# wdc3iii/legged_gym_dev

Hardware: AMD Instinct MI355X
Metric: env-steps/sec (whole node), ANYmal-C flat 4096 envs per GPU (higher is better)
Workload: dtype f32

## Files before the change

legged_gym_dev_amd/csrc/ppo_api.hip:

```cpp
#include <cstdlib>
#include <cstring>
#include <string>
#include <vector>

#include "ppo_device.h"
#include "ppo_mlp_args.h"
#include "ppo_rnn.h"

void lg_set_error(const std::string &s);

extern "C" {
void ppok_gemm_fwd(const GemmArgs *g, int nz, hipStream_t s);
void ppok_gemm_dx(const GemmArgs *g, int nz, hipStream_t s);
void ppok_sync_planes(const PpoDev *P, hipStream_t s);
int ppok_mlp_fwd(const MlpArgs *g, const PpoDev *P, hipStream_t s);
int ppok_mlp_supported(const MlpArgs *g);
int64_t ppok_mlp_frag_elems(int K, int N);
void ppok_mlp_frag_build(const MlpArgs *g, hipStream_t s);
void ppok_gemm_dw(const GemmArgs *g, int nz, hipStream_t s);
void ppok_act_sample(const PpoDev *P, const float *obs, const float *cobs, const float *mu, const float *val, int t,
                     int64_t cnt, int inject, hipStream_t s);
void ppok_process_step(const PpoDev *P, const float *rew, const uint8_t *dones, const uint8_t *tos, int t, hipStream_t s);
void ppok_gae(const PpoDev *P, const float *last_values, hipStream_t s);
void ppok_det_fold(const PpoDev *P, hipStream_t s);
void ppok_adv_normalize(const PpoDev *P, hipStream_t s);
void ppok_gather(const PpoDev *P, int mb, hipStream_t s);
void ppok_randperm(const PpoDev *P, int n, uint64_t update_idx, hipStream_t s);
void ppok_loss(const PpoDev *P, const float *mu, const float *v, float *dmu, float *dval, hipStream_t s);
int ppok_step(const PpoDev *P, int par, const PpoDev *G, int gather_mb, hipStream_t s);
// ... 62 lines not shown
    long long *det_buf;
    int act_code;
    int grads_dirty;
    lg_ctx *env;
    int pp_pending, pp_t, pp_use_tos;
    int params_dirty;
    int fused_act;
    MlpArgs mlp;
    int step, inject;
    int64_t act_count, update_count;
    int Mmax;
    std::vector<void *> allocs;
    int64_t perm_count;
    struct MbSet { float *obs, *critic_obs, *actions, *mu, *scalars; } mbset[2];
    int mb_cur, mb_ready, mb_last;
    lg_ppo_buffers pub;
    Rnn rnn;
};

template <typename T>
static bool palloc(lg_ppo *p, T **out, size_t n) {
    void *q = nullptr;
    size_t bytes = (n ? n : 1) * sizeof(T);
    if (hipMalloc(&q, bytes) != hipSuccess || hipMemset(q, 0, bytes) != hipSuccess) return false;
    p->allocs.push_back(q);
    *out = (T *)q;
    return true;
}
#define PA(ptr, n) do { if (!palloc(p, &(ptr), (n))) { lg_set_error("hipMalloc failed in lg_ppo_create"); lg_ppo_destroy(p); return -100; } } while (0)

// ... 44 lines not shown
        bufs[n] = p->dev.grads + p->dev.num_params; counts[n++] = 2;
    }
    return n;
}
static void reduce_layer_bucket(lg_ppo *p, int l, hipStream_t ready_on) {
    float *bufs[4];
    int64_t counts[4];
    const int n = bucket_extents(p, l, bufs, counts);
    hipStream_t cs = lg_comm_stream_(p->comm);
    (void)hipEventRecord(p->ev_bucket, ready_on);
    (void)hipStreamWaitEvent(cs, p->ev_bucket, 0);
    const int rc = lg_comm_group_allreduce_(p->comm, bufs, counts, n, cs);
    if (rc && !p->comm_rc) p->comm_rc = rc;
}

static void backward(lg_ppo *p, int M, const float *in0, const float *in1, int skip_head = 0) {
    const float *in[2] = {in0, in1};
    auto det_args = [&](GemmArgs &g) {
        g.det_base = p->dev.grads; g.det64 = p->dev.det64; g.det_n = p->dev.num_params + 2;
    };
    const int nl = p->net[0].nl;
    for (int l = nl - 1 - skip_head; l >= 0; --l) {
        GemmArgs g;
        memset(&g, 0, sizeof(g));
        det_args(g);
        for (int z = 0; z < 2; ++z) {
            Net &n = p->net[z];
            g.A[z] = n.dz[l + 1]; g.lda[z] = n.dims[l + 1];
            g.B[z] = l == 0 ? in[z] : n.act[l]; g.ldb[z] = n.dims[l];
            g.C[z] = p->dev.grads + n.w_off[l]; g.ldc[z] = n.dims[l];
            g.M[z] = n.dims[l + 1]; g.N[z] = n.dims[l]; g.K[z] = M;
            if (l == 0 && !p->rnn.H) {
                const int ldp = z == 0 ? p->dev.Op : p->dev.OCp;
                g.ldb[z] = ldp;
                if (ldp != n.dims[0]) { g.N[z] = ldp; g.nstore[z] = n.dims[0]; }
            }
        }
        const bool on_side = p->overlap && l > 0;
        hipStream_t dw_stream = on_side ? p->side : p->stream;
        if (on_side) {
            (void)hipEventRecord(p->ev_dz, p->stream);
            (void)hipStreamWaitEvent(p->side, p->ev_dz, 0);
        }
        ppok_gemm_dw(&g, 2, dw_stream);
        if (p->comm) reduce_layer_bucket(p, l, dw_stream);
        if (l > 0) {
            memset(&g, 0, sizeof(g));
            det_args(g);
            for (int z = 0; z < 2; ++z) {
                Net &n = p->net[z];
                g.A[z] = n.dz[l + 1]; g.lda[z] = n.dims[l + 1];
                g.B[z] = p->dev.params + n.w_off[l]; g.ldb[z] = n.dims[l];
                g.Bpl[z] = p->dev.wpl + n.pl_off[l];
                g.C[z] = n.dz[l]; g.ldc[z] = n.dims[l];
                g.aux[z] = n.act[l]; g.ldaux[z] = n.dims[l];
                g.colsum[z] = p->dev.grads + n.b_off[l - 1];
                g.M[z] = M; g.N[z] = n.dims[l]; g.K[z] = n.dims[l + 1];
// ... 6 lines not shown
    if (p->rnn.H) {
        GemmArgs g;
        memset(&g, 0, sizeof(g));
        for (int z = 0; z < 2; ++z) {
            Net &n = p->net[z];
            g.A[z] = n.dz[1]; g.lda[z] = n.dims[1];
            g.B[z] = p->dev.params + n.w_off[0]; g.ldb[z] = n.dims[0];
            g.Bpl[z] = p->dev.wpl + n.pl_off[0];
            g.C[z] = p->rnn.dh[z]; g.ldc[z] = n.dims[0];
            g.aux[z] = p->rnn.dh[z]; g.ldaux[z] = n.dims[0];
            g.M[z] = M; g.N[z] = n.dims[0]; g.K[z] = n.dims[1];
        }
        g.elu = 0;
        g.pl_stride = p->dev.pl_stride;
        ppok_gemm_dx(&g, 2, p->stream);
    }
    if (p->overlap) {
        (void)hipEventRecord(p->ev_side, p->side);
        (void)hipStreamWaitEvent(p->stream, p->ev_side, 0);
    }
    if (p->comm) {
        const bool rec = p->comm_timing && p->comm_ev_used + 2 <= 2 * 4096;
        if (rec) {
            while (p->comm_ev.size() < p->comm_ev_used + 2) { hipEvent_t e; (void)hipEventCreate(&e); p->comm_ev.push_back(e); }
            (void)hipEventRecord(p->comm_ev[p->comm_ev_used], p->stream);
        }
        (void)hipEventRecord(lg_comm_event_(p->comm), lg_comm_stream_(p->comm));
        (void)hipStreamWaitEvent(p->stream, lg_comm_event_(p->comm), 0);
        if (rec) { (void)hipEventRecord(p->comm_ev[p->comm_ev_used + 1], p->stream); p->comm_ev_used += 2; }
    }
// ... 162 lines not shown
    const int OC = cfg->num_critic_obs > 0 ? cfg->num_critic_obs : O;
    if ((long)N * T % cfg->num_mini_batches != 0 && (long)N * T / cfg->num_mini_batches == 0) { lg_set_error("bad minibatch count"); return -5; }
    const int H = rc ? rc->hidden : 0;
    if (rc) {
        if (rc->type != 0) { lg_set_error("recurrent policy: only rnn_type 'lstm' (0) is implemented"); return -6; }
        if (rc->layers != 1) { lg_set_error("recurrent policy: only rnn_num_layers = 1 is implemented"); return -6; }
        if (H < 32 || H > 512 || H % 32) { lg_set_error("recurrent policy: rnn_hidden_size must be a multiple of 32 in [32, 512]"); return -6; }
    }
    lg_ppo *p = new lg_ppo();
    p->cfg = *cfg;
    memset(&p->rnn, 0, sizeof(p->rnn));
    p->stream = nullptr;
    p->act_code = cfg->activation + 1;
    p->fused_act = getenv("LG_FUSED_ACT") ? atoi(getenv("LG_FUSED_ACT")) : 1;
    p->overlap = getenv("LG_PPO_OVERLAP") ? atoi(getenv("LG_PPO_OVERLAP")) : 1;
    if (hipStreamCreateWithFlags(&p->side, hipStreamNonBlocking) != hipSuccess ||
        hipEventCreateWithFlags(&p->ev_dz, hipEventDisableTiming) != hipSuccess ||
        hipEventCreateWithFlags(&p->ev_side, hipEventDisableTiming) != hipSuccess ||
        hipEventCreateWithFlags(&p->ev_bucket, hipEventDisableTiming) != hipSuccess) {
        lg_set_error("stream/event creation failed"); delete p; return -100;
    }
    p->step = 0; p->inject = 0; p->act_count = 0; p->update_count = 0; p->params_dirty = 1;
    p->comm = nullptr; p->comm_rc = 0; p->comm_timing = 0; p->comm_ev_used = 0;
    p->env = nullptr; p->pp_pending = 0;
    p->perm_count = 0;
    const int R = (int)((long)N * T / cfg->num_mini_batches);
    p->Mmax = R > N ? R : N;

    int64_t off = 0;
    PpoDev &d = p->dev;
    memset(&d, 0, sizeof(d));
    d.off_std = (int)off; off += A;
    for (int z = 0; z < 2; ++z) {
// ... 65 lines not shown
    if (cfg->num_critic_obs > 0) PA(d.st_critic_obs, TN * OC); else d.st_critic_obs = d.st_obs;
    PA(d.st_actions, TN * A); PA(d.st_rewards, TN); PA(d.st_values, TN); PA(d.st_returns, TN); PA(d.st_adv, TN);
    PA(d.st_log_prob, TN); PA(d.st_mu, TN * A); PA(d.st_sigma, A); PA(d.st_dones, TN);
    PA(d.act_actions, (size_t)N * A); PA(d.act_values, N); PA(d.act_log_prob, N); PA(d.act_mu, (size_t)N * A);
    PA(d.stats, 8); PA(d.loss_acc, 4); PA(d.noise, (size_t)N * A); PA(d.perm, TN); PA(d.adv_partial, 4);
    for (int k = 0; k < 2; ++k) {
        lg_ppo::MbSet &m = p->mbset[k];
        PA(m.obs, (size_t)R * d.Op);
        if (cfg->num_critic_obs > 0) PA(m.critic_obs, (size_t)R * d.OCp); else m.critic_obs = m.obs;
        PA(m.actions, (size_t)R * A); PA(m.mu, (size_t)R * A); PA(m.scalars, (size_t)R * 4);
    }
    p->mb_cur = 0; p->mb_ready = -1; p->mb_last = -1;
    d.mb_obs = p->mbset[0].obs; d.mb_critic_obs = p->mbset[0].critic_obs; d.mb_actions = p->mbset[0].actions;
    d.mb_mu = p->mbset[0].mu; d.mb_scalars = p->mbset[0].scalars;
    PA(d.head_part, ppok_head_part_floats());
    PA(d.cur_reward_sum, N); PA(d.cur_episode_len, N); PA(d.ep_stats, 4); PA(d.ep_ring, 200); PA(d.ep_ring_count, 1);
    for (int z = 0; z < 2; ++z) {
        Net &n = p->net[z];
        n.act[0] = nullptr; n.dz[0] = nullptr;
        for (int l = 1; l <= n.nl; ++l) { PA(n.act[l], (size_t)p->Mmax * n.dims[l]); PA(n.dz[l], (size_t)p->Mmax * n.dims[l]); }
    }
    if (H) {
        Rnn &q = p->rnn;
        const size_t NH = (size_t)N * H, Rr = (size_t)R;
        for (int z = 0; z < 2; ++z) {
            PA(q.h[z], NH); PA(q.c[z], NH); PA(q.sv_h[z], TN * H); PA(q.sv_c[z], TN * H); PA(q.tmp_h[z], NH); PA(q.tmp_c[z], NH);
            PA(q.pg[z], Rr * 4 * H); PA(q.gates[z], Rr * 4 * H);
            PA(q.hout[z], Rr * H); PA(q.cout[z], Rr * H); PA(q.hused[z], Rr * H); PA(q.cused[z], Rr * H); PA(q.dh[z], Rr * H);
            PA(q.dc[z], (size_t)q.mbs * H);
        }
// ... 54 lines not shown
    }
    out->hidden = p->rnn.H;
    return 0;
}
int lg_ppo_reset_hidden(lg_ppo *p, const uint8_t *dones) {
    if (!p->rnn.H) { lg_set_error("lg_ppo_reset_hidden: not a recurrent learner"); return -15; }
    flush_rollout_epilogue(p);
    const Rnn &q = p->rnn;
    ppok_lstm_reset(q.h[0], q.c[0], q.h[1], q.c[1], dones, p->cfg.num_envs, q.H, p->stream);
    return launch_ok();
}
int lg_ppo_get_buffers(lg_ppo *p, lg_ppo_buffers *out) { *out = p->pub; return 0; }
int lg_ppo_set_stream(lg_ppo *p, void *s) { p->stream = (hipStream_t)s; return 0; }
int lg_ppo_inject_noise(lg_ppo *p, int enable) { p->inject = enable; return 0; }
int lg_ppo_debug_set_overlap(lg_ppo *p, int v) { p->overlap = v; return 0; }
int lg_ppo_debug_set_fused_act(lg_ppo *p, int v) { p->fused_act = v && p->mlp.wfrag; return 0; }
int lg_ppo_debug_get_fused_act(lg_ppo *p) { return p->fused_act; }
int lg_ppo_debug_set_act_count(lg_ppo *p, long long v) { p->act_count = v; return 0; }

int lg_ppo_param_layout(lg_ppo *p, int64_t *offsets, int64_t *shapes, int max_entries) {
    int k = 0;
    auto put = [&](int64_t o, int64_t r, int64_t c) {
        if (k < max_entries) { offsets[k] = o; shapes[2 * k] = r; shapes[2 * k + 1] = c; }
        ++k;
    };
    put(p->dev.off_std, p->cfg.num_actions, 0);
    for (int z = 0; z < 2; ++z)
        for (int l = 0; l < p->net[z].nl; ++l) {
            put(p->net[z].w_off[l], p->net[z].dims[l + 1], p->net[z].dims[l]);
            put(p->net[z].b_off[l], p->net[z].dims[l + 1], 0);
// ... 40 lines not shown
            g.pp_t = p->pp_t; g.pp_use_tos = p->pp_use_tos;
            g.pp_env = lg_internal_take_finalize(p->env, &g.pp_counter);
            p->pp_pending = 0;
        } else flush_rollout_epilogue(p);
        fused = ppok_mlp_fwd(&g, &p->dev, p->stream);
        if (fused != 0 && g.pp) { lg_set_error("fused act launch refused with a rollout epilogue attached"); return -13; }
        if (fused == 0) {
            p->act_count++;
            const int rc = launch_ok();
            if (rc == 0) p->params_dirty = 0;
            return rc;
        }
    }
    if (!p->fused_act) flush_rollout_epilogue(p);
    if (fused != 0) {
        if (dirty) ppok_sync_planes(&p->dev, p->stream);
        const float *in0 = obs, *in1 = cobs;
        if (p->rnn.H) {
            rnn_stash_live(p, 3, p->step);
            rnn_live_step(p, 3, obs, cobs, p->step);
            in0 = p->rnn.h[0]; in1 = p->rnn.h[1];
        }
        forward(p, p->cfg.num_envs, in0, in1, 3, 0, true);
    }
    ppok_act_sample(&p->dev, obs, cobs, p->net[0].act[p->net[0].nl], p->net[1].act[p->net[1].nl], p->step, p->act_count,
                    p->inject, p->stream);
    p->act_count++;
    const int rc = launch_ok();
    if (rc == 0) p->params_dirty = 0;
    return rc;
}
// ... 36 lines not shown
    if (!p->rnn.H || p->cfg.num_envs % p->cfg.num_mini_batches == 0) return 0;
    lg_set_error("recurrent policy: the update needs num_envs to be a multiple of num_mini_batches (its minibatches are whole envs)");
    return 1;
}

int lg_ppo_begin_update(lg_ppo *p) {
    if (rnn_update_refused(p)) return -6;
    flush_rollout_epilogue(p);
    const size_t n = (size_t)p->dev.mb_rows * p->cfg.num_mini_batches;
    if (!p->rnn.H) ppok_randperm(&p->dev, (int)n, (uint64_t)p->perm_count++, p->stream);
    p->mb_ready = -1;
    (void)hipMemsetAsync(p->dev.stats + 2, 0, 2 * sizeof(float), p->stream);
    (void)hipMemsetAsync(p->dev.stats + 5, 0, sizeof(float), p->stream);
    (void)hipMemsetAsync(p->dev.loss_acc, 0, 4 * sizeof(float), p->stream);
    p->grads_dirty = 1;
    ppok_sync_planes(&p->dev, p->stream);
    return launch_ok();
}

int lg_ppo_minibatch_backward(lg_ppo *p, int epoch, int mb) {
    (void)epoch;
    if (rnn_update_refused(p)) return -6;
    PpoDev &d = p->dev;
    const int R = d.mb_rows;
    if (p->grads_dirty) (void)hipMemsetAsync(d.grads, 0, (size_t)(d.num_params + 2) * sizeof(float), p->stream);
    p->grads_dirty = 1;
    auto use_set = [&](PpoDev &dev, int k) {
        const lg_ppo::MbSet &m = p->mbset[k];
        dev.mb_obs = m.obs; dev.mb_critic_obs = m.critic_obs; dev.mb_actions = m.actions; dev.mb_mu = m.mu; dev.mb_scalars = m.scalars;
    };
    if (p->mb_ready == mb) {
        p->mb_cur ^= 1;
        use_set(d, p->mb_cur);
    } else {
        ppok_gather(&d, mb, p->stream);
    }
    p->mb_ready = -1;
    p->mb_last = mb;
    Net &na = p->net[0], &nc = p->net[1];
    const int nl = na.nl, H3 = na.dims[nl - 1];
    const bool fuse = p->act_code == 1 && nl >= 2 && nc.dims[nl - 1] == H3 && (H3 == 128 || H3 == 64 || H3 == 32);
    if (p->rnn.H) {
        rnn_forward_seq(p, mb);
        forward(p, R, p->rnn.hout[0], p->rnn.hout[1], 3, fuse ? 1 : 0, true, false);
    } else
        forward(p, R, d.mb_obs, d.mb_critic_obs, 3, fuse ? 1 : 0, true, true);
    if (fuse) {
        ppok_head_fused(&d, H3, na.act[nl - 1], nc.act[nl - 1], na.dz[nl - 1], nc.dz[nl - 1], na.w_off[nl - 1], na.b_off[nl - 1],
                        nc.w_off[nl - 1], nc.b_off[nl - 1], na.b_off[nl - 2], nc.b_off[nl - 2], p->stream);
    } else {
        ppok_loss(&d, na.act[na.nl], nc.act[nc.nl], na.dz[na.nl], nc.dz[nc.nl], p->stream);
    }
    if (fuse && p->comm) reduce_layer_bucket(p, nl - 1, p->stream);
    if (p->rnn.H) {
        backward(p, R, p->rnn.hout[0], p->rnn.hout[1], fuse ? 1 : 0);
        rnn_backward_seq(p, mb);
    } else
        backward(p, R, d.mb_obs, d.mb_critic_obs, fuse ? 1 : 0);
    if (d.det64) ppok_det_fold(&d, p->stream);
    if (p->comm_rc) { const int rc = p->comm_rc; p->comm_rc = 0; return rc; }
    return launch_ok();
}

int lg_ppo_minibatch_step(lg_ppo *p) {
    int next = -1;
    PpoDev other = p->dev;
    if (p->cfg.num_mini_batches > 1 && p->mb_last >= 0) {
        next = (p->mb_last + 1) % p->cfg.num_mini_batches;
        const lg_ppo::MbSet &m = p->mbset[p->mb_cur ^ 1];
        other.mb_obs = m.obs; other.mb_critic_obs = m.critic_obs; other.mb_actions = m.actions; other.mb_mu = m.mu; other.mb_scalars = m.scalars;
    }
    if (ppok_step(&p->dev, (int)(p->update_count & 1), &other, next, p->stream)) p->mb_ready = next;
    p->mb_last = -1;
    p->grads_dirty = 0;
    p->params_dirty = 1;
    p->update_count++;
    return launch_ok();
}

int lg_ppo_end_update(lg_ppo *p) { p->step = 0; return 0; }

int lg_ppo_set_comm(lg_ppo *p, lg_comm *c) {
    if (c && p->rnn.H) { lg_set_error("lg_ppo_set_comm: the per-layer gradient buckets do not cover the LSTM of a recurrent learner; reduce the whole gradient buffer between lg_ppo_minibatch_backward and lg_ppo_minibatch_step instead"); return -14; }
    if (c && p->dev.det64) { lg_set_error("gradient buckets inside the backward pass cannot be combined with deterministic mode"); return -14; }
    p->comm = c;
    return 0;
}
// ... 61 lines not shown
```

legged_gym_dev_amd/csrc/ppo_device.h:

```cpp
#pragma once
#include "lg_device.h"

#define LG_PPO_MAX_A 16
#define LG_PPO_MAX_LAYERS (LG_MAX_HIDDEN + 1)

struct GemmArgs {
    const float *A[2], *B[2], *bias[2], *aux[2];
    float *C[2], *colsum[2];
    int M[2], N[2], K[2], lda[2], ldb[2], ldc[2], ldaux[2];
    int elu;
    const uint16_t *Bpl[2];
    int64_t pl_stride;
    int Kpl[2], ldbpl[2];
    int nstore[2];
    const float *det_base;
    long long *det64;
    int64_t det_n;
};

#define LG_PPO_MAX_SEG (2 * LG_PPO_MAX_LAYERS)

struct PpoDev {
    int N, T, A, O, OC, mb_rows, world, env_offset;
    int adaptive, clipped_value;
    uint64_t seed;
    float gamma, lam, clip, value_coef, entropy_coef, desired_kl, max_grad_norm;
    int64_t num_params;
    int off_std, off_bias_actor_head, off_bias_critic_head;
    float *params, *grads, *adam_m, *adam_v;
    float *st_obs, *st_critic_obs, *st_actions, *st_rewards, *st_values, *st_returns, *st_adv, *st_log_prob, *st_mu, *st_sigma;
    uint8_t *st_dones;
    float *act_actions, *act_values, *act_log_prob, *act_mu;
// ... 2 lines not shown
    float *noise;
    int32_t *perm;
    float *adv_partial;
    float *mb_obs, *mb_critic_obs, *mb_actions, *mb_mu, *mb_scalars;
    int Op, OCp;
    float *cur_reward_sum, *cur_episode_len, *ep_stats, *ep_ring;
    int32_t *ep_ring_count;
    float *head_part;
    uint16_t *wpl;
    int32_t *pl_dest;
    int64_t pl_stride;
    int nseg;
    int64_t seg_off[LG_PPO_MAX_SEG], seg_pl[LG_PPO_MAX_SEG];
    int seg_rows[LG_PPO_MAX_SEG], seg_cols[LG_PPO_MAX_SEG];
    long long *det64;
};

#define LG_DET_SCALE 1099511627776.0
__device__ __forceinline__ void det_add64(long long *q, float v) {
    atomicAdd(reinterpret_cast<unsigned long long *>(q), (unsigned long long)__double2ll_rn((double)v * LG_DET_SCALE));
}
__device__ __forceinline__ void acc_add(const PpoDev &P, float *p, float v) {
    if (!P.det64) { atomicAdd(p, v); return; }
    long long i;
    if (p >= P.grads && p < P.grads + P.num_params + 2) i = p - P.grads;
    else if (p >= P.loss_acc && p < P.loss_acc + 4) i = P.num_params + 2 + (p - P.loss_acc);
    else i = P.num_params + 6 + (p - P.adv_partial);
    det_add64(P.det64 + i, v);
}
__device__ __forceinline__ void acc_add(const GemmArgs &g, float *p, float v) {
// ... 33 lines not shown
```

legged_gym_dev_amd/csrc/ppo_gemm.hip:

```cpp
#include <cstring>
#include <type_traits>

#include "ppo_device.h"
#include "ppo_split_bf16.h"

__device__ __forceinline__ void xcd_tile(int lin, int inner, int outer, int &o, int &i) {
    if ((outer & 7) == 0) {
        const int c = lin & 7, j = lin >> 3;
        o = c + 8 * (j / inner);
        i = j % inner;
    } else {
        o = lin / inner;
        i = lin % inner;
    }
}

#define BK 32

struct GemmTiles { int z, M, N, K, tiles_n, tiles_m; };
template <int BM, int BN>
__device__ __forceinline__ bool gemm_tiles(const GemmArgs &g, GemmTiles &t) {
    t.z = blockIdx.z;
    t.M = g.M[t.z]; t.N = g.N[t.z]; t.K = g.K[t.z];
    t.tiles_n = (t.N + BN - 1) / BN; t.tiles_m = (t.M + BM - 1) / BM;
// ... 506 lines not shown
    for (int v = 0; v < NV; ++v) {
        const int idx = threadIdx.x + v * NT;
        const int c = idx & (ROWS / 4 - 1), r = idx / (ROWS / 4);
        const bool in = (mask >> v) & 1u;
        const float x0 = in ? regs[v].x : 0.f, x1 = in ? regs[v].y : 0.f, x2 = in ? regs[v].z : 0.f, x3 = in ? regs[v].w : 0.f;
        uint32_t h0, m0, l0, h1, m1, l1;
        split2(x0, x1, h0, m0, l0);
        split2(x2, x3, h1, m1, l1);
        unsigned char *d = lds + plt_off<ROWS>(r, c >> 1) + 8 * (c & 1);
        *reinterpret_cast<uint2 *>(d) = make_uint2(h0, h1);
        *reinterpret_cast<uint2 *>(d + PL) = make_uint2(m0, m1);
        *reinterpret_cast<uint2 *>(d + 2 * PL) = make_uint2(l0, l1);
    }
}

template <int TM, int TN, int WGM, int WGN, int PD = 2>
__global__ void __launch_bounds__(64 * WGM * WGN, WGM * WGN == 8 ? 4 : 2) k_gemm_dw_t(GemmArgs g) {
    constexpr int BM = 32 * TM * WGM, BN = 32 * TN * WGN, NT = 64 * WGM * WGN;
    constexpr int APL = plt_plane_bytes<BM>(), BPL = plt_plane_bytes<BN>();
    constexpr int NVA = BM * BK / 4 / NT, NVB = BN * BK / 4 / NT;
    GemmTiles t;
    if (!gemm_tiles<BM, BN>(g, t)) return;
    const int z = t.z, M = t.M, N = t.N;
    int slice, tile;
    xcd_tile((int)(blockIdx.x + gridDim.x * blockIdx.y), (int)gridDim.x, (int)gridDim.y, slice, tile);
    const int m0 = (tile / t.tiles_n) * BM, n0 = (tile % t.tiles_n) * BN;
    int k_begin, k_end;
    if (!k_slice(t.K, slice, k_begin, k_end)) return;
    const float *__restrict__ A = g.A[z];
    const float *__restrict__ B = g.B[z];
    const int lda = g.lda[z], ldb = g.ldb[z], ldc = g.ldc[z];
    __shared__ __attribute__((aligned(16))) unsigned char lds[3 * (APL + BPL)];
// ... 59 lines not shown
                stage_store_x6t<BM, NT>(lds, na, nma);
                stage_store_x6t<BN, NT>(lds_b, nb, nmb);
            }
            lds_barrier();
        };
        for (int k0 = k_begin; k0 < k_end; k0 += PD * BK) {
    #pragma unroll
            for (int d = 0; d < PD; ++d)
                if (d == 0 || k0 + d * BK < k_end)
                    body(k0 + d * BK, ra[d], rb[d], ma[d], mb[d], ra[(d + 1) % PD], rb[(d + 1) % PD], ma[(d + 1) % PD], mb[(d + 1) % PD]);
        }
    };
    if (a_vec && b_vec) run(std::true_type{});
    else run(std::false_type{});
    GEMM_EPILOGUE(2, TM, TN, BM, BN, g, z, M, g.nstore[z] ? g.nstore[z] : N, m0, n0, wm, wn, li, lk, ldc, acc);
}

static int g_gemm_x6 = 1;
extern "C" void ppok_debug_set_x6(int v) { g_gemm_x6 = v != 0; }

#include "ppo_gemm_glds.h"

struct GemmShape { int maxM, maxN; unsigned small_tiles, big_tiles; bool big; };
static GemmShape gemm_shape(const GemmArgs &g, int nz, int splits) {
    GemmShape sh{0, 0, 0, 0, false};
    for (int z = 0; z < nz; ++z) { sh.maxM = g.M[z] > sh.maxM ? g.M[z] : sh.maxM; sh.maxN = g.N[z] > sh.maxN ? g.N[z] : sh.maxN; }
    const long big_tiles = (long)((sh.maxM + 127) / 128) * ((sh.maxN + 127) / 128);
    sh.small_tiles = (unsigned)(((sh.maxM + 63) / 64) * ((sh.maxN + 63) / 64));
    sh.big_tiles = (unsigned)big_tiles;
    sh.big = big_tiles * splits >= 192 && sh.maxN > 64 && sh.maxM > 64;
// ... 64 lines not shown
    GemmArgs gp = *g;
    for (int z = 0; z < nz; ++z) {
        if (g->Kpl[z]) gp.K[z] = g->Kpl[z];
        if (g->ldbpl[z]) gp.ldb[z] = g->ldbpl[z];
    }
    if (planes_ok(gp, nz, &GemmArgs::K)) launch_gemm_pl<0>(gp, nz, s);
    else if (g_gemm_x6) launch_gemm<true, true, 0>(*g, nz, s);
    else launch_gemm_ref<true, true, 0>(*g, nz, 1, s);
}
extern "C" void ppok_gemm_dx(const GemmArgs *g, int nz, hipStream_t s) {
    if (planes_ok(*g, nz, &GemmArgs::N)) launch_gemm_pl<1, false, 2>(*g, nz, s);
    else if (g_gemm_x6) launch_gemm<true, false, 1>(*g, nz, s);
    else launch_gemm_ref<true, false, 1>(*g, nz, 1, s);
}
extern "C" void ppok_gemm_dw(const GemmArgs *g, int nz, hipStream_t s) { launch_gemm_dw(*g, nz, dw_splits(*g, nz), s); }

extern "C" void ppok_debug_gemm(const float *A, const float *B, float *C, int M, int N, int K, int mode, int splits, void *stream) {
    GemmArgs g;
    memset(&g, 0, sizeof(g));
    g.A[0] = A; g.B[0] = B; g.C[0] = C; g.M[0] = M; g.N[0] = N; g.K[0] = K; g.ldc[0] = N;
    if (mode == 0) { g.lda[0] = K; g.ldb[0] = K; ppok_gemm_fwd(&g, 1, (hipStream_t)stream); }
    else if (mode == 1) { g.lda[0] = K; g.ldb[0] = N; g.aux[0] = C; g.ldaux[0] = N; g.elu = 1; ppok_gemm_dx(&g, 1, (hipStream_t)stream); }
    else { g.lda[0] = M; g.ldb[0] = N; launch_gemm_dw(g, 1, splits, (hipStream_t)stream); }
}

__global__ void __launch_bounds__(256) k_debug_split(const float *__restrict__ W, uint16_t *__restrict__ pl, int64_t n, int64_t stride) {
    for (int64_t k = blockIdx.x * (int64_t)blockDim.x + threadIdx.x; k < n; k += (int64_t)gridDim.x * blockDim.x) {
        uint32_t h, m, l;
        split2(W[k], 0.f, h, m, l);
        pl[k] = (uint16_t)h; pl[stride + k] = (uint16_t)m; pl[2 * stride + k] = (uint16_t)l;
// ... 21 lines not shown
```

legged_gym_dev_amd/csrc/ppo_kernels.hip:

```cpp
#include <type_traits>

#include "ppo_device.h"
#include "ppo_split_bf16.h"

__global__ void k_act_sample(PpoDev P, const float *__restrict__ obs, const float *__restrict__ critic_obs,
                             const float *__restrict__ mu, const float *__restrict__ val, int t, int64_t act_count, int inject) {
    const int i = blockIdx.x * blockDim.x + threadIdx.x;
    const int N = P.N, A = P.A, O = P.O;
    if (t >= 0) {
        const size_t tot = (size_t)N * O, step = (size_t)gridDim.x * blockDim.x;
        for (size_t k = i; k < tot; k += step) P.st_obs[(size_t)t * tot + k] = obs[k];
        if (P.st_critic_obs != P.st_obs) {
            const size_t totc = (size_t)N * P.OC;
            for (size_t k = i; k < totc; k += step) P.st_critic_obs[(size_t)t * totc + k] = critic_obs[k];
        }
    }
    const float *std = P.params + P.off_std;
    if (i < A && t == 0) P.st_sigma[i] = std[i];
    if (i >= N) return;
    float lp = 0.f;
    for (int a = 0; a < A; ++a) {
        float m = mu[(size_t)i * A + a], s = std[a];
        float z = inject ? P.noise[(size_t)i * A + a] : philox_normal(P.seed, (uint32_t)(P.env_offset + i), (uint64_t)act_count, a);
        float act = m + s * z;
// ... 709 lines not shown
    for (int64_t i = blockIdx.x * (int64_t)blockDim.x + threadIdx.x; i < n; i += (int64_t)gridDim.x * blockDim.x) {
        const long long q = P.det64[i];
        if (q == 0) continue;
        float *t = i < P.num_params + 2 ? P.grads + i : i < P.num_params + 6 ? P.loss_acc + (i - P.num_params - 2) : P.adv_partial + (i - P.num_params - 6);
        *t += (float)((double)q * (1.0 / LG_DET_SCALE));
        P.det64[i] = 0;
    }
}
__device__ __forceinline__ void write_planes(const PpoDev &P, int64_t k, float x) {
    const int d = P.pl_dest[k];
    if (d < 0) return;
    uint32_t h, m, l;
    split2(x, 0.f, h, m, l);
    P.wpl[d] = (uint16_t)h; P.wpl[P.pl_stride + d] = (uint16_t)m; P.wpl[2 * P.pl_stride + d] = (uint16_t)l;
}
__global__ void __launch_bounds__(256) k_sync_planes(PpoDev P) {
    for (int64_t k = blockIdx.x * (int64_t)blockDim.x + threadIdx.x; k < P.num_params; k += (int64_t)gridDim.x * blockDim.x)
        write_planes(P, k, P.params[k]);
}
__global__ void __launch_bounds__(256) k_opt_adam(PpoDev P, int par) {
    const float total = sqrtf(P.loss_acc[2 + par]);
    const float coef = fminf(P.max_grad_norm / (total + 1e-6f), 1.0f);
    const float lr = P.stats[0], t = P.stats[4];
    const float bc1 = 1.0f - powf(0.9f, t), bc2 = 1.0f - powf(0.999f, t);
    const float inv_world = 1.0f / (float)P.world;
    for (int64_t k = blockIdx.x * (int64_t)blockDim.x + threadIdx.x; k < P.num_params; k += (int64_t)gridDim.x * blockDim.x) {
        const float g = P.grads[k] * inv_world * coef;
        const float m = 0.9f * P.adam_m[k] + 0.1f * g;
        const float v = 0.999f * P.adam_v[k] + 0.001f * g * g;
        P.adam_m[k] = m;
        P.adam_v[k] = v;
        const float pn = P.params[k] - (lr / bc1) * m / (sqrtf(v) / sqrtf(bc2) + 1e-8f);
        P.params[k] = pn;
        P.grads[k] = 0.f;
        write_planes(P, k, pn);
    }
    if (blockIdx.x == 0 && threadIdx.x == 0) {
        P.grads[P.num_params] = 0.f; P.grads[P.num_params + 1] = 0.f;
        P.loss_acc[2 + (par ^ 1)] = 0.f;
    }
}

extern "C" {
void ppok_act_sample(const PpoDev *P, const float *obs, const float *cobs, const float *mu, const float *val, int t,
                     int64_t cnt, int inject, hipStream_t s) {
    const int blocks = (P->N + 63) / 64;
    hipLaunchKernelGGL(k_act_sample, dim3(blocks > 256 ? blocks : 256), dim3(64), 0, s, *P, obs, cobs, mu, val, t, cnt, inject);
}
void ppok_process_step(const PpoDev *P, const float *rew, const uint8_t *dones, const uint8_t *tos, int t, hipStream_t s) {
    hipLaunchKernelGGL(k_process_step, dim3((P->N + 255) / 256), dim3(256), 0, s, *P, rew, dones, tos, t);
}
void ppok_det_fold(const PpoDev *P, hipStream_t s) { hipLaunchKernelGGL(k_det_fold, dim3(512), dim3(256), 0, s, *P); }
void ppok_gae(const PpoDev *P, const float *last_values, hipStream_t s) {
    (void)hipMemsetAsync(P->adv_partial, 0, 3 * sizeof(float), s);
    hipLaunchKernelGGL(k_gae, dim3((P->N + 255) / 256), dim3(256), 0, s, *P, last_values);
    if (P->det64) ppok_det_fold(P, s);
// ... 23 lines not shown
        if (P->A <= 12)
            hipLaunchKernelGGL((k_head_net<128, 12>), dim3(nrows, 2), block, 0, s, *P, xa, xc, dza, dzc, P->params + w_a, P->params + w_c, b_a, b_c);
        else
            hipLaunchKernelGGL((k_head_net<128, LG_PPO_MAX_A>), dim3(nrows, 2), block, 0, s, *P, xa, xc, dza, dzc, P->params + w_a, P->params + w_c, b_a, b_c);
        constexpr int NTOT = HEAD_PART_STRIDE(128);
        hipLaunchKernelGGL((k_head_finish<128>), dim3((NTOT + 255) / 256, HEAD_FIN_CHUNKS, 2), block, 0, s, *P, nrows, w_a, b_a, w_c, b_c,
                           b_prev_a, b_prev_c);
    } else if (H3 == 64) hipLaunchKernelGGL((k_head_fused<64>), grid, block, 0, s, *P, xa, xc, dza, dzc, w_a, b_a, w_c, b_c, b_prev_a, b_prev_c);
    else if (H3 == 32) hipLaunchKernelGGL((k_head_fused<32>), grid, block, 0, s, *P, xa, xc, dza, dzc, w_a, b_a, w_c, b_c, b_prev_a, b_prev_c);
    else return -1;
    return 0;
}
void ppok_loss(const PpoDev *P, const float *mu, const float *v, float *dmu, float *dval, hipStream_t s) {
    hipLaunchKernelGGL(k_loss, dim3((P->mb_rows + 255) / 256), dim3(256), 0, s, *P, mu, v, dmu, dval);
}
void ppok_sync_planes(const PpoDev *P, hipStream_t s) { hipLaunchKernelGGL(k_sync_planes, dim3(256), dim3(256), 0, s, *P); }
int ppok_step(const PpoDev *P, int par, const PpoDev *G, int gather_mb, hipStream_t s) {
    const bool g4 = gather_mb >= 0 && (P->A & 3) == 0;
    const int gblocks = g4 ? (P->mb_rows * 32 + 255) / 256 : 0;
    hipLaunchKernelGGL(k_opt_prepare, dim3(128 + gblocks), dim3(256), 0, s, *P, par, 128, g4 ? *G : *P, gather_mb);
    if (P->det64) ppok_det_fold(P, s);
    constexpr int adam_max = 1024;
    const long want = (P->num_params + 255) / 256;
    hipLaunchKernelGGL(k_opt_adam, dim3((unsigned)(want < adam_max ? (want > 0 ? want : 1) : adam_max)), dim3(256), 0, s, *P, par);
    return g4 ? 1 : 0;
}
}
```

legged_gym_dev_amd/lib.py:

```python
import ctypes as C
import os
import subprocess

import numpy as np

from . import capi

_DIR = os.path.dirname(os.path.abspath(__file__))
SO_PATH = os.environ.get("LG_HIP_LIB") or os.path.join(_DIR, "lib", "liblegged_hip.so")
_lib = None


class LeggedHipError(RuntimeError):
    pass


def build(force=False):
    src = os.path.join(_DIR, "csrc")
    if force and os.path.isfile(SO_PATH):
        os.remove(SO_PATH)
    subprocess.check_call(["make", "-C", src, "-s", "-j4"])
    return SO_PATH


# ... 27 lines not shown
    lib.lg_ppo_process_env_step.argtypes = [vp, vp, vp, vp]
    lib.lg_ppo_compute_returns.argtypes = [vp, vp]
    lib.lg_ppo_normalize_advantages.argtypes = [vp]
    lib.lg_ppo_begin_update.argtypes = [vp]
    lib.lg_ppo_minibatch_backward.argtypes = [vp, C.c_int, C.c_int]
    lib.lg_ppo_minibatch_step.argtypes = [vp]
    lib.lg_ppo_end_update.argtypes = [vp]
    lib.lg_ppo_act_inference.argtypes = [vp, vp, vp, C.c_int64]
    lib.lg_ppo_params_changed.argtypes = [vp]
    lib.lg_ppo_set_deterministic.argtypes = [vp, C.c_int]
    lib.lg_ppo_attach_env.argtypes = [vp, vp]
    lib.lg_ppo_create_recurrent.argtypes = [C.POINTER(capi.lg_ppo_cfg), C.POINTER(capi.lg_ppo_rnn_cfg), C.POINTER(vp)]
    lib.lg_ppo_get_rnn_buffers.argtypes = [vp, C.POINTER(capi.lg_ppo_rnn_buffers)]
    lib.lg_ppo_reset_hidden.argtypes = [vp, vp]
    lib.lg_ppo_debug_bucket_extents.argtypes = [vp, C.c_int, C.POINTER(C.c_int64), C.POINTER(C.c_int64)]


_TORCH_DT = {"f4": "float32", "u1": "uint8", "i8": "int64", "i4": "int32"}


class _DevArray:

    def __init__(self, ptr, shape, typestr, owner):
        self.__cuda_array_interface__ = {"data": (int(ptr), False), "shape": tuple(int(s) for s in shape),
                                         "typestr": typestr, "version": 2, "strides": None}
        self._owner = owner


def device_tensor(ptr, shape, dt, owner, device):
    import torch
# ... 66 lines not shown
```

Before: 7.086 million.

## Fuse gradient-norm reduction into dW GEMM tails and single-kernel Adam step

The dW GEMM now counts finished K-slices per output tile with atomic tickets. The last slice to finish for a tile computes that tile's squared gradient norm, and one tile also folds in the bias and std gradients, so the clip norm is ready when backward ends. A new single-pass optimizer kernel then applies clipping, adaptive LR and Adam, writes the weight planes, and uses ping-pong slots. This replaces the separate norm reduction and multi-stage step, and the next minibatch gather moves onto the side stream. The edge events also drop the system fence. The change adds tickets, atomics and a path that is only valid for single-GPU, non-recurrent, non-deterministic configurations, and it relaxes the launch bounds to allow more waves.

```diff
diff --git a/legged_gym_dev_amd/csrc/ppo_api.hip b/legged_gym_dev_amd/csrc/ppo_api.hip
--- a/legged_gym_dev_amd/csrc/ppo_api.hip
+++ b/legged_gym_dev_amd/csrc/ppo_api.hip
@@ -12,7 +12,10 @@
 extern "C" {
 void ppok_gemm_fwd(const GemmArgs *g, int nz, hipStream_t s);
 void ppok_gemm_dx(const GemmArgs *g, int nz, hipStream_t s);
-void ppok_sync_planes(const PpoDev *P, hipStream_t s);
+void ppok_sync_planes(const PpoDev *P, int par, hipStream_t s);
+void ppok_opt_sync_slots(const PpoDev *P, int par, hipStream_t s);
+void ppok_step_fused(const PpoDev *P, int par, hipStream_t s);
+int ppok_gemm_dw_tickets();
 int ppok_mlp_fwd(const MlpArgs *g, const PpoDev *P, hipStream_t s);
 int ppok_mlp_supported(const MlpArgs *g);
 int64_t ppok_mlp_frag_elems(int K, int N);
@@ -105,6 +108,13 @@
     int64_t perm_count;
     struct MbSet { float *obs, *critic_obs, *actions, *mu, *scalars; } mbset[2];
     int mb_cur, mb_ready, mb_last;
+    int opt_fused;
+    int norm_ready;
+    int slots_stale;
+    long long fused_steps;
+    uint32_t *tickets;
+    size_t n_tickets;
+    int64_t tk_off[LG_PPO_MAX_LAYERS][2];
     lg_ppo_buffers pub;
     Rnn rnn;
 };
@@ -179,8 +189,15 @@
     if (rc && !p->comm_rc) p->comm_rc = rc;
 }
 
-static void backward(lg_ppo *p, int M, const float *in0, const float *in1, int skip_head = 0) {
+static bool opt_fused_now(const lg_ppo *p) {
+    return p->opt_fused && !p->dev.det64 && !p->comm && !p->rnn.H && p->dev.world == 1 && p->tickets && ppok_gemm_dw_tickets() &&
+           p->dev.num_params < (1ll << 31);
+}
+
+static void backward(lg_ppo *p, int M, const float *in0, const float *in1, int skip_head = 0, bool take_norm = false, int par = 0,
+                     const PpoDev *other = nullptr, int gather_mb = -1) {
     const float *in[2] = {in0, in1};
+    bool side_edge = false;
     auto det_args = [&](GemmArgs &g) {
         g.det_base = p->dev.grads; g.det64 = p->dev.det64; g.det_n = p->dev.num_params + 2;
     };
@@ -200,12 +217,28 @@
                 g.ldb[z] = ldp;
                 if (ldp != n.dims[0]) { g.N[z] = ldp; g.nstore[z] = n.dims[0]; }
             }
+            if (take_norm) g.ticket[z] = p->tickets + p->tk_off[l][z];
+        }
+        if (take_norm) {
+            g.normsq = p->dev.opt_slots + par; g.norm_scale = 1.0f / (float)p->dev.world;
+            if (l == 0) {
+                auto put = [&](int64_t off, int64_t cnt) { g.xoff[g.nx] = (int)off; g.xcnt[g.nx] = (int)cnt; ++g.nx; };
+                g.xbase = p->dev.grads;
+                put(p->dev.off_std, p->cfg.num_actions);
+                for (int z = 0; z < 2; ++z) {
+                    Net &n = p->net[z];
+                    for (int k = 0; k < nl; ++k) put(n.b_off[k], n.dims[k + 1]);
+                    if (skip_head) put(n.w_off[nl - 1], (int64_t)n.dims[nl] * n.dims[nl - 1]);
+                }
+                g.xcopy_from = p->dev.grads + p->dev.num_params; g.xcopy_to = p->dev.opt_slots + 6 + par;
+            }
         }
         const bool on_side = p->overlap && l > 0;
         hipStream_t dw_stream = on_side ? p->side : p->stream;
         if (on_side) {
             (void)hipEventRecord(p->ev_dz, p->stream);
             (void)hipStreamWaitEvent(p->side, p->ev_dz, 0);
+            side_edge = true;
         }
         ppok_gemm_dw(&g, 2, dw_stream);
         if (p->comm) reduce_layer_bucket(p, l, dw_stream);
@@ -242,6 +275,10 @@
         g.elu = 0;
         g.pl_stride = p->dev.pl_stride;
         ppok_gemm_dx(&g, 2, p->stream);
+    }
+    if (gather_mb >= 0) {
+        if (p->overlap && !side_edge) { (void)hipEventRecord(p->ev_dz, p->stream); (void)hipStreamWaitEvent(p->side, p->ev_dz, 0); }
+        ppok_gather(other, gather_mb, p->overlap ? p->side : p->stream);
     }
     if (p->overlap) {
         (void)hipEventRecord(p->ev_side, p->side);
@@ -434,9 +471,16 @@
     p->act_code = cfg->activation + 1;
     p->fused_act = getenv("LG_FUSED_ACT") ? atoi(getenv("LG_FUSED_ACT")) : 1;
     p->overlap = getenv("LG_PPO_OVERLAP") ? atoi(getenv("LG_PPO_OVERLAP")) : 1;
+    p->opt_fused = getenv("LG_PPO_OPT_FUSED") ? atoi(getenv("LG_PPO_OPT_FUSED")) : 1;
+    p->norm_ready = 0; p->slots_stale = 1; p->fused_steps = 0; p->tickets = nullptr; p->n_tickets = 0;
+#ifdef LG_EV_SYSTEM_FENCE
+    const unsigned edge_flags = hipEventDisableTiming;
+#else
+    const unsigned edge_flags = hipEventDisableTiming | hipEventDisableSystemFence;
+#endif
     if (hipStreamCreateWithFlags(&p->side, hipStreamNonBlocking) != hipSuccess ||
-        hipEventCreateWithFlags(&p->ev_dz, hipEventDisableTiming) != hipSuccess ||
-        hipEventCreateWithFlags(&p->ev_side, hipEventDisableTiming) != hipSuccess ||
+        hipEventCreateWithFlags(&p->ev_dz, edge_flags) != hipSuccess ||
+        hipEventCreateWithFlags(&p->ev_side, edge_flags) != hipSuccess ||
         hipEventCreateWithFlags(&p->ev_bucket, hipEventDisableTiming) != hipSuccess) {
         lg_set_error("stream/event creation failed"); delete p; return -100;
     }
@@ -532,6 +576,19 @@
     d.mb_obs = p->mbset[0].obs; d.mb_critic_obs = p->mbset[0].critic_obs; d.mb_actions = p->mbset[0].actions;
     d.mb_mu = p->mbset[0].mu; d.mb_scalars = p->mbset[0].scalars;
     PA(d.head_part, ppok_head_part_floats());
+    PA(d.opt_slots, 8);
+    if (!H) {
+        size_t nt = 0;
+        for (int l = 0; l < p->net[0].nl; ++l)
+            for (int z = 0; z < 2; ++z) {
+                const Net &n = p->net[z];
+                const int cols = l == 0 ? (z == 0 ? d.Op : d.OCp) : n.dims[l];
+                p->tk_off[l][z] = (int64_t)nt;
+                nt += (size_t)((n.dims[l + 1] + 63) / 64) * ((cols + 63) / 64);
+            }
+        PA(p->tickets, nt);
+        p->n_tickets = nt;
+    }
     PA(d.cur_reward_sum, N); PA(d.cur_episode_len, N); PA(d.ep_stats, 4); PA(d.ep_ring, 200); PA(d.ep_ring_count, 1);
     for (int z = 0; z < 2; ++z) {
         Net &n = p->net[z];
@@ -616,6 +673,12 @@
 int lg_ppo_set_stream(lg_ppo *p, void *s) { p->stream = (hipStream_t)s; return 0; }
 int lg_ppo_inject_noise(lg_ppo *p, int enable) { p->inject = enable; return 0; }
 int lg_ppo_debug_set_overlap(lg_ppo *p, int v) { p->overlap = v; return 0; }
+int lg_ppo_debug_set_opt_fused(lg_ppo *p, int v) { p->opt_fused = v != 0; return 0; }
+long long lg_ppo_debug_opt_fused_steps(lg_ppo *p) { return p->fused_steps; }
+long long lg_ppo_debug_opt_chain_buffers(lg_ppo *p, void **tickets, void **slots, void **planes, long long *pl_stride) {
+    *tickets = p->tickets; *slots = p->dev.opt_slots; *planes = p->dev.wpl; *pl_stride = p->dev.pl_stride;
+    return (long long)p->n_tickets;
+}
 int lg_ppo_debug_set_fused_act(lg_ppo *p, int v) { p->fused_act = v && p->mlp.wfrag; return 0; }
 int lg_ppo_debug_get_fused_act(lg_ppo *p) { return p->fused_act; }
 int lg_ppo_debug_set_act_count(lg_ppo *p, long long v) { p->act_count = v; return 0; }
@@ -686,7 +749,7 @@
     }
     if (!p->fused_act) flush_rollout_epilogue(p);
     if (fused != 0) {
-        if (dirty) ppok_sync_planes(&p->dev, p->stream);
+        if (dirty) ppok_sync_planes(&p->dev, -1, p->stream);
         const float *in0 = obs, *in1 = cobs;
         if (p->rnn.H) {
             rnn_stash_live(p, 3, p->step);
@@ -753,7 +816,8 @@
     (void)hipMemsetAsync(p->dev.stats + 5, 0, sizeof(float), p->stream);
     (void)hipMemsetAsync(p->dev.loss_acc, 0, 4 * sizeof(float), p->stream);
     p->grads_dirty = 1;
-    ppok_sync_planes(&p->dev, p->stream);
+    ppok_sync_planes(&p->dev, (int)(p->update_count & 1), p->stream);
+    p->slots_stale = 0;
     return launch_ok();
 }
 
@@ -762,8 +826,16 @@
     if (rnn_update_refused(p)) return -6;
     PpoDev &d = p->dev;
     const int R = d.mb_rows;
-    if (p->grads_dirty) (void)hipMemsetAsync(d.grads, 0, (size_t)(d.num_params + 2) * sizeof(float), p->stream);
+    if (p->grads_dirty) {
+        (void)hipMemsetAsync(d.grads, 0, (size_t)(d.num_params + 2) * sizeof(float), p->stream);
+        if (p->tickets) {
+            (void)hipMemsetAsync(p->tickets, 0, p->n_tickets * sizeof(uint32_t), p->stream);
+            (void)hipMemsetAsync(d.opt_slots, 0, 2 * sizeof(float), p->stream);
+        }
+    }
     p->grads_dirty = 1;
+    const bool take_norm = opt_fused_now(p);
+    const int par = (int)(p->update_count & 1);
     auto use_set = [&](PpoDev &dev, int k) {
         const lg_ppo::MbSet &m = p->mbset[k];
         dev.mb_obs = m.obs; dev.mb_critic_obs = m.critic_obs; dev.mb_actions = m.actions; dev.mb_mu = m.mu; dev.mb_scalars = m.scalars;
@@ -794,8 +866,15 @@
     if (p->rnn.H) {
         backward(p, R, p->rnn.hout[0], p->rnn.hout[1], fuse ? 1 : 0);
         rnn_backward_seq(p, mb);
-    } else
-        backward(p, R, d.mb_obs, d.mb_critic_obs, fuse ? 1 : 0);
+    } else {
+        PpoDev other = d;
+        const int next = (mb + 1) % p->cfg.num_mini_batches;
+        const bool ahead = take_norm && p->cfg.num_mini_batches > 1 && (d.A & 3) == 0;
+        if (ahead) use_set(other, p->mb_cur ^ 1);
+        backward(p, R, d.mb_obs, d.mb_critic_obs, fuse ? 1 : 0, take_norm, par, &other, ahead ? next : -1);
+        if (ahead) p->mb_ready = next;
+    }
+    p->norm_ready = take_norm;
     if (d.det64) ppok_det_fold(&d, p->stream);
     if (p->comm_rc) { const int rc = p->comm_rc; p->comm_rc = 0; return rc; }
     return launch_ok();
@@ -804,12 +883,27 @@
 int lg_ppo_minibatch_step(lg_ppo *p) {
     int next = -1;
     PpoDev other = p->dev;
-    if (p->cfg.num_mini_batches > 1 && p->mb_last >= 0) {
+    const int par = (int)(p->update_count & 1);
+    if (p->norm_ready && opt_fused_now(p)) {
+        if (p->slots_stale) { ppok_opt_sync_slots(&p->dev, par, p->stream); p->slots_stale = 0; }
+        ppok_step_fused(&p->dev, par, p->stream);
+        p->fused_steps++;
+        p->norm_ready = 0;
+        p->mb_last = -1;
+        p->grads_dirty = 0;
+        p->params_dirty = 1;
+        p->update_count++;
+        return launch_ok();
+    }
+    if (p->norm_ready) (void)hipMemsetAsync(p->dev.opt_slots, 0, 2 * sizeof(float), p->stream);
+    p->norm_ready = 0;
+    p->slots_stale = 1;
+    if (p->cfg.num_mini_batches > 1 && p->mb_last >= 0 && p->mb_ready < 0) {
         next = (p->mb_last + 1) % p->cfg.num_mini_batches;
         const lg_ppo::MbSet &m = p->mbset[p->mb_cur ^ 1];
         other.mb_obs = m.obs; other.mb_critic_obs = m.critic_obs; other.mb_actions = m.actions; other.mb_mu = m.mu; other.mb_scalars = m.scalars;
     }
-    if (ppok_step(&p->dev, (int)(p->update_count & 1), &other, next, p->stream)) p->mb_ready = next;
+    if (ppok_step(&p->dev, par, &other, next, p->stream)) p->mb_ready = next;
     p->mb_last = -1;
     p->grads_dirty = 0;
     p->params_dirty = 1;
diff --git a/legged_gym_dev_amd/csrc/ppo_device.h b/legged_gym_dev_amd/csrc/ppo_device.h
--- a/legged_gym_dev_amd/csrc/ppo_device.h
+++ b/legged_gym_dev_amd/csrc/ppo_device.h
@@ -4,6 +4,7 @@
 #define LG_PPO_MAX_A 16
 #define LG_PPO_MAX_LAYERS (LG_MAX_HIDDEN + 1)
 
+#define LG_GEMM_MAX_X (2 * LG_PPO_MAX_LAYERS + 3)
 struct GemmArgs {
     const float *A[2], *B[2], *bias[2], *aux[2];
     float *C[2], *colsum[2];
@@ -16,6 +17,14 @@
     const float *det_base;
     long long *det64;
     int64_t det_n;
+    uint32_t *ticket[2];
+    float *normsq;
+    float norm_scale;
+    const float *xbase;
+    int nx;
+    int xoff[LG_GEMM_MAX_X], xcnt[LG_GEMM_MAX_X];
+    const float *xcopy_from;
+    float *xcopy_to;
 };
 
 #define LG_PPO_MAX_SEG (2 * LG_PPO_MAX_LAYERS)
@@ -48,6 +57,7 @@
     int64_t seg_off[LG_PPO_MAX_SEG], seg_pl[LG_PPO_MAX_SEG];
     int seg_rows[LG_PPO_MAX_SEG], seg_cols[LG_PPO_MAX_SEG];
     long long *det64;
+    float *opt_slots;
 };
 
 #define LG_DET_SCALE 1099511627776.0
diff --git a/legged_gym_dev_amd/csrc/ppo_gemm.hip b/legged_gym_dev_amd/csrc/ppo_gemm.hip
--- a/legged_gym_dev_amd/csrc/ppo_gemm.hip
+++ b/legged_gym_dev_amd/csrc/ppo_gemm.hip
@@ -544,8 +544,53 @@
     }
 }
 
+template <int BM, int BN, int NT>
+__device__ __forceinline__ void dw_norm_arrive(const GemmArgs &g, int z, int M, int N, int K, int m0, int n0, int tile, int ldc,
+                                               unsigned char *scratch) {
+    uint32_t *drawn = reinterpret_cast<uint32_t *>(scratch);
+    float *red = reinterpret_cast<float *>(scratch) + 4;
+    const int per = ((K + (int)gridDim.y - 1) / (int)gridDim.y + BK - 1) / BK * BK;
+    const uint32_t slices = (uint32_t)((K + per - 1) / per);
+    asm volatile("s_waitcnt vmcnt(0)" ::: "memory");
+    __syncthreads();
+    if (threadIdx.x == 0) *drawn = atomicAdd(&g.ticket[z][tile], 1u);
+    __syncthreads();
+    if (*drawn != slices - 1) return;
+    __builtin_amdgcn_fence(__ATOMIC_ACQUIRE, "agent");
+    const float *C = g.C[z];
+    const float sc = g.norm_scale;
+    const int rows = min(BM, M - m0), cols = min(BN, N - n0);
+    float s = 0.f;
+    for (int i = threadIdx.x; i < BM * BN; i += NT) {
+        const int r = i / BN, c = i % BN;
+        if (r < rows && c < cols) {
+            const float v = __hip_atomic_load(&C[(size_t)(m0 + r) * ldc + n0 + c], __ATOMIC_RELAXED, __HIP_MEMORY_SCOPE_AGENT) * sc;
+            s += v * v;
+        }
+    }
+    const bool rider = z == 0 && tile == 0 && g.xbase;
+    if (rider) {
+        for (int x = 0; x < g.nx; ++x)
+            for (int k = threadIdx.x; k < g.xcnt[x]; k += NT) {
+                const float v = __hip_atomic_load(&g.xbase[g.xoff[x] + k], __ATOMIC_RELAXED, __HIP_MEMORY_SCOPE_AGENT) * sc;
+                s += v * v;
+            }
+    }
+#pragma unroll
+    for (int w = 32; w > 0; w >>= 1) s += __shfl_xor(s, w);
+    if ((threadIdx.x & 63) == 0) red[threadIdx.x >> 6] = s;
+    __syncthreads();
+    if (threadIdx.x == 0) {
+        float tot = 0.f;
+        for (int w = 0; w < NT / 64; ++w) tot += red[w];
+        acc_add(g, g.normsq, tot);
+        __hip_atomic_store(&g.ticket[z][tile], 0u, __ATOMIC_RELAXED, __HIP_MEMORY_SCOPE_AGENT);
+        if (rider && g.xcopy_to) *g.xcopy_to = __hip_atomic_load(g.xcopy_from, __ATOMIC_RELAXED, __HIP_MEMORY_SCOPE_AGENT);
+    }
+}
+
 template <int TM, int TN, int WGM, int WGN, int PD = 2>
-__global__ void __launch_bounds__(64 * WGM * WGN, WGM * WGN == 8 ? 4 : 2) k_gemm_dw_t(GemmArgs g) {
+__global__ void __launch_bounds__(64 * WGM * WGN, 4) k_gemm_dw_t(GemmArgs g) {
     constexpr int BM = 32 * TM * WGM, BN = 32 * TN * WGN, NT = 64 * WGM * WGN;
     constexpr int APL = plt_plane_bytes<BM>(), BPL = plt_plane_bytes<BN>();
     constexpr int NVA = BM * BK / 4 / NT, NVB = BN * BK / 4 / NT;
@@ -635,6 +680,7 @@
     if (a_vec && b_vec) run(std::true_type{});
     else run(std::false_type{});
     GEMM_EPILOGUE(2, TM, TN, BM, BN, g, z, M, g.nstore[z] ? g.nstore[z] : N, m0, n0, wm, wn, li, lk, ldc, acc);
+    if (g.ticket[z]) dw_norm_arrive<BM, BN, NT>(g, z, M, g.nstore[z] ? g.nstore[z] : N, t.K, m0, n0, tile, ldc, lds);
 }
 
 static int g_gemm_x6 = 1;
@@ -729,6 +775,7 @@
     else launch_gemm_ref<true, false, 1>(*g, nz, 1, s);
 }
 extern "C" void ppok_gemm_dw(const GemmArgs *g, int nz, hipStream_t s) { launch_gemm_dw(*g, nz, dw_splits(*g, nz), s); }
+extern "C" int ppok_gemm_dw_tickets() { return g_gemm_x6; }
 
 extern "C" void ppok_debug_gemm(const float *A, const float *B, float *C, int M, int N, int K, int mode, int splits, void *stream) {
     GemmArgs g;
diff --git a/legged_gym_dev_amd/csrc/ppo_kernels.hip b/legged_gym_dev_amd/csrc/ppo_kernels.hip
--- a/legged_gym_dev_amd/csrc/ppo_kernels.hip
+++ b/legged_gym_dev_amd/csrc/ppo_kernels.hip
@@ -747,7 +747,8 @@
     split2(x, 0.f, h, m, l);
     P.wpl[d] = (uint16_t)h; P.wpl[P.pl_stride + d] = (uint16_t)m; P.wpl[2 * P.pl_stride + d] = (uint16_t)l;
 }
-__global__ void __launch_bounds__(256) k_sync_planes(PpoDev P) {
+__global__ void __launch_bounds__(256) k_sync_planes(PpoDev P, int par) {
+    if (par >= 0 && blockIdx.x == 0 && threadIdx.x == 0) { P.opt_slots[2 + par] = P.stats[0]; P.opt_slots[4 + par] = P.stats[4]; }
     for (int64_t k = blockIdx.x * (int64_t)blockDim.x + threadIdx.x; k < P.num_params; k += (int64_t)gridDim.x * blockDim.x)
         write_planes(P, k, P.params[k]);
 }
@@ -773,6 +774,46 @@
         P.loss_acc[2 + (par ^ 1)] = 0.f;
     }
 }
+
+__global__ void __launch_bounds__(256) k_opt_step(PpoDev P, int par) {
+    const float *sl = P.opt_slots;
+    const float kl = sl[6 + par] / ((float)P.mb_rows * (float)P.world);
+    float lr = sl[2 + par];
+    if (P.adaptive) {
+        if (kl > P.desired_kl * 2.0f) lr = fmaxf(1e-5f, lr / 1.5f);
+        else if (kl < P.desired_kl / 2.0f && kl > 0.0f) lr = fminf(1e-2f, lr * 1.5f);
+    }
+    const float t = sl[4 + par] + 1.0f;
+    const float total = sqrtf(sl[par]);
+    const float coef = fminf(P.max_grad_norm / (total + 1e-6f), 1.0f);
+    const float bc1 = 1.0f - powf(0.9f, t), bc2 = 1.0f - powf(0.999f, t);
+    const float inv_world = 1.0f / (float)P.world;
+    for (int64_t k = blockIdx.x * (int64_t)blockDim.x + threadIdx.x; k < P.num_params; k += (int64_t)gridDim.x * blockDim.x) {
+        const float g = P.grads[k] * inv_world * coef;
+        const float m = 0.9f * P.adam_m[k] + 0.1f * g;
+        const float v = 0.999f * P.adam_v[k] + 0.001f * g * g;
+        P.adam_m[k] = m;
+        P.adam_v[k] = v;
+        const float pn = P.params[k] - (lr / bc1) * m / (sqrtf(v) / sqrtf(bc2) + 1e-8f);
+        P.params[k] = pn;
+        P.grads[k] = 0.f;
+        write_planes(P, k, pn);
+    }
+    if (blockIdx.x == 0 && threadIdx.x == 0) {
+        P.stats[0] = lr;
+        P.stats[1] = kl;
+        P.stats[2] += P.loss_acc[0] / (float)P.mb_rows;
+        P.stats[3] += P.loss_acc[1] / (float)P.mb_rows;
+        P.stats[4] = t;
+        P.stats[5] += 1.0f;
+        P.loss_acc[0] = 0.f; P.loss_acc[1] = 0.f;
+        P.grads[P.num_params] = 0.f; P.grads[P.num_params + 1] = 0.f;
+        P.opt_slots[par ^ 1] = 0.f;
+        P.opt_slots[2 + (par ^ 1)] = lr;
+        P.opt_slots[4 + (par ^ 1)] = t;
+    }
+}
+__global__ void k_opt_sync_slots(PpoDev P, int par) { P.opt_slots[2 + par] = P.stats[0]; P.opt_slots[4 + par] = P.stats[4]; }
 
 extern "C" {
 void ppok_act_sample(const PpoDev *P, const float *obs, const float *cobs, const float *mu, const float *val, int t,
@@ -826,7 +867,12 @@
 void ppok_loss(const PpoDev *P, const float *mu, const float *v, float *dmu, float *dval, hipStream_t s) {
     hipLaunchKernelGGL(k_loss, dim3((P->mb_rows + 255) / 256), dim3(256), 0, s, *P, mu, v, dmu, dval);
 }
-void ppok_sync_planes(const PpoDev *P, hipStream_t s) { hipLaunchKernelGGL(k_sync_planes, dim3(256), dim3(256), 0, s, *P); }
+void ppok_sync_planes(const PpoDev *P, int par, hipStream_t s) { hipLaunchKernelGGL(k_sync_planes, dim3(256), dim3(256), 0, s, *P, par); }
+void ppok_opt_sync_slots(const PpoDev *P, int par, hipStream_t s) { hipLaunchKernelGGL(k_opt_sync_slots, dim3(1), dim3(1), 0, s, *P, par); }
+void ppok_step_fused(const PpoDev *P, int par, hipStream_t s) {
+    const long want = (P->num_params + 255) / 256;
+    hipLaunchKernelGGL(k_opt_step, dim3((unsigned)(want < 1024 ? (want > 0 ? want : 1) : 1024)), dim3(256), 0, s, *P, par);
+}
 int ppok_step(const PpoDev *P, int par, const PpoDev *G, int gather_mb, hipStream_t s) {
     const bool g4 = gather_mb >= 0 && (P->A & 3) == 0;
     const int gblocks = g4 ? (P->mb_rows * 32 + 255) / 256 : 0;
diff --git a/legged_gym_dev_amd/lib.py b/legged_gym_dev_amd/lib.py
--- a/legged_gym_dev_amd/lib.py
+++ b/legged_gym_dev_amd/lib.py
@@ -65,6 +65,12 @@
     lib.lg_ppo_get_rnn_buffers.argtypes = [vp, C.POINTER(capi.lg_ppo_rnn_buffers)]
     lib.lg_ppo_reset_hidden.argtypes = [vp, vp]
     lib.lg_ppo_debug_bucket_extents.argtypes = [vp, C.c_int, C.POINTER(C.c_int64), C.POINTER(C.c_int64)]
+    if hasattr(lib, "lg_ppo_debug_set_opt_fused"):
+        lib.lg_ppo_debug_set_opt_fused.argtypes = [vp, C.c_int]
+        lib.lg_ppo_debug_opt_fused_steps.argtypes = [vp]
+        lib.lg_ppo_debug_opt_fused_steps.restype = C.c_longlong
+        lib.lg_ppo_debug_opt_chain_buffers.argtypes = [vp, C.POINTER(vp), C.POINTER(vp), C.POINTER(vp), C.POINTER(C.c_longlong)]
+        lib.lg_ppo_debug_opt_chain_buffers.restype = C.c_longlong
 
 
 _TORCH_DT = {"f4": "float32", "u1": "uint8", "i8": "int64", "i4": "int32"}
```

New measurement: 7.072 million. No clear change (-0.2%).
